# GenkiK/monodepth2

Hardware: AMD Instinct MI355X
Metric: training images/sec at 640x192 mono, 1/2/4/8 GPUs; loss delta vs ref (higher is better)
Workload: dtype f32; 1 GPU; mono_640x192 ResNet-18 batch=12/GPU full train step (configs[1]); global_batch=12, height=192, width=640, parallelism=dp1, step=hipgraph replay

## Files before the change

### include/md2hot.h

```cpp
#ifndef MD2HOT_H
#define MD2HOT_H

#include <stddef.h>
#include <stdint.h>

#ifdef __cplusplus
extern "C" {
#endif

#define MD2_ABI_VERSION 24
#define MD2_MAX_SCALES 4
#define MD2_MAX_SRC 3

#define MD2_OK 0
#define MD2_ERR_ARG (-1)
#define MD2_ERR_HIP (-2)

#define MD2_NO_SSIM          (1u << 0)
#define MD2_AVG_REPROJECTION (1u << 1)
#define MD2_NO_AUTOMASK      (1u << 2)
#define MD2_V1_MULTISCALE    (1u << 3)
#define MD2_T_PER_SCALE      (1u << 4)
#define MD2_PREDICTIVE_MASK  (1u << 5)

// ... 165 lines not shown
    uint8_t reserved;
    uint8_t order[4];
    float brightness, contrast, saturation;
} md2_aug_item;

typedef struct md2_aug_plan md2_aug_plan;

md2_aug_plan* md2_aug_plan_create(const md2_aug_desc* desc);
void md2_aug_plan_destroy(md2_aug_plan* plan);

int md2_aug_run(md2_aug_plan* plan, const uint8_t* frames, const md2_aug_item* items,
                float* const* color, float* const* color_aug, void* stream);
int md2_aug_run2(md2_aug_plan* plan, const uint8_t* frames, const md2_aug_item* items,
                 float* const* color, float* const* color_aug, uint32_t* src8, void* stream);

md2_aug_plan* md2_aug_plan_create_mixed(const md2_aug_desc* desc, const int32_t* sizes, int num_sizes);
int md2_aug_run_mixed(md2_aug_plan* plan, const uint8_t* frames_base, uint64_t total_bytes,
                      const int32_t* item_class, const uint64_t* frame_offset, const md2_aug_item* items,
                      float* const* color, float* const* color_aug, uint32_t* src8, void* stream);

#define MD2_BN_RELU     (1u << 0)
#define MD2_BN_RESIDUAL (1u << 1)
#define MD2_BN_BF16     (1u << 2)

typedef struct md2_bn_desc {
    int64_t pixels;
    int32_t channels;
    uint32_t flags;
    float eps, momentum;
    int32_t groups;
    int32_t reserved;
} md2_bn_desc;

size_t md2_bn_workspace_bytes(const md2_bn_desc* desc);
int md2_bn_fwd(const md2_bn_desc* desc, const void* x, const float* gamma, const float* beta,
               const void* residual, float* running_mean, float* running_var, void* y,
               float* save_mean, float* save_invstd, void* workspace, void* stream);
int md2_bn_bwd(const md2_bn_desc* desc, const void* x, const void* y, const void* grad_y,
               const float* gamma, const float* save_mean, const float* save_invstd,
               void* grad_x, void* grad_residual, float* grad_gamma, float* grad_beta,
               void* workspace, void* stream);
int md2_bn_bwd_multi(const md2_bn_desc* desc, const void* x, const void* y, const void* grad_y,
                     const void* grad_y2, const void* grad_y3, const float* gamma, const float* save_mean,
                     const float* save_invstd, void* grad_x, void* grad_residual, float* grad_gamma,
                     float* grad_beta, void* workspace, void* stream);
int md2_bn_fwd_mask(const md2_bn_desc* desc, const void* x, const float* gamma, const float* beta,
// ... 116 lines not shown

typedef struct md2_viz_desc {
    int32_t batch;
    int32_t in_height, in_width;
    int32_t out_height, out_width;
    int32_t percentile;
    uint32_t flags;
    int32_t reserved;
} md2_viz_desc;

size_t md2_disp_colorize_workspace_bytes(const md2_viz_desc* desc);
int md2_disp_colorize(const md2_viz_desc* desc, const float* disp, uint8_t* rgb, float* resized, float* stats,
                      void* workspace, void* stream);

int md2_bn_pool_fwd_supported(const md2_bn_desc* desc, int height, int width);
int md2_bn_pool_fwd(const md2_bn_desc* desc, int height, int width, const float* x, const float* gamma,
                    const float* beta, float* running_mean, float* running_var, float* y, uint8_t* relu_mask,
                    float* pooled, uint32_t* idx, float* save_mean, float* save_invstd, void* workspace,
                    void* stream);
int md2_bn_bwd_reduce_mask(const md2_bn_desc* desc, const void* x, const uint8_t* relu_mask, const void* grad_y,
                           const float* gamma, const float* save_mean, const float* save_invstd, float* grad_gamma,
                           float* grad_beta, void* workspace, void* stream);
size_t md2_bn_coef_offset(const md2_bn_desc* desc);
int md2_stem_wgrad_bn_supported(const md2_stem_desc* desc);
int md2_stem_wgrad_bn(const md2_stem_desc* desc, const float* x, const float* grad, const float* z,
                      const uint8_t* relu_mask, const float* save_mean, const float* coef, int bn_groups,
                      float* grad_weight, void* workspace, void* stream);

#define MD2_DEPTH16_POST_PROCESS (1u << 0)

typedef struct md2_depth16_desc {
    int32_t batch;
    int32_t in_height, in_width;
    int32_t out_height, out_width;
    uint32_t flags;
    double min_depth, max_depth;
    double scale_factor;
    double clip_max;
    double quant;
    int64_t reserved;
} md2_depth16_desc;

int md2_depth_export16_check(const md2_depth16_desc* desc);
int md2_depth_export16(const md2_depth16_desc* desc, const float* disp, const float* disp_flipped, uint16_t* out,
                       void* stream);

// ... 5 lines not shown
```

### monodepth2_amd/_lib.py

```python
from __future__ import annotations

import ctypes
import os
import threading

import torch

from .build import LIB_PATH as _BUILT_LIB
from .build import source_hash

LIB_PATH = os.environ.get("MD2_LIB", _BUILT_LIB)

MAX_SCALES = 4
MAX_SRC = 3
ABI_VERSION = 24

NO_SSIM = 1 << 0
AVG_REPROJECTION = 1 << 1
NO_AUTOMASK = 1 << 2
V1_MULTISCALE = 1 << 3
T_PER_SCALE = 1 << 4
PREDICTIVE_MASK = 1 << 5

_vp = ctypes.c_void_p
# ... 23 lines not shown
_lib = None

EXPORTS = ["md2_abi_version", "md2_last_error", "md2_workspace_bytes", "md2_select_bytes",
           "md2_photometric_fwd", "md2_photometric_bwd", "md2_generate_images", "md2_tiebreak_noise",
           "md2_timing_begin", "md2_timing_end", "md2_timing_calls", "md2_decoder_pad_fwd", "md2_decoder_pad_bwd",
           "md2_decoder_pad_workspace_bytes", "md2_adam_step", "md2_adam_step_dev", "md2_adam_hyper", "md2_adam_apply_dev", "md2_encoder_input",
           "md2_pose_fwd", "md2_pose_bwd", "md2_aug_plan_create", "md2_aug_plan_destroy", "md2_aug_run",
           "md2_bn_workspace_bytes", "md2_bn_fwd", "md2_bn_bwd", "md2_maxpool3s2_fwd", "md2_maxpool3s2_bwd",
           "md2_disp_head_workspace_bytes", "md2_disp_head_fwd", "md2_disp_head_bwd",
           "md2_stem_wgrad_workspace_bytes", "md2_stem_wgrad", "md2_stem_fwd", "md2_conv_col2im", "md2_bias_act_fwd", "md2_bias_act_bwd",
           "md2_bias_act_workspace_bytes", "md2_maxpool3s2_bwd_add", "md2_bn_bwd_multi",
           "md2_conv_fwd", "md2_conv_workspace_bytes", "md2_conv_split_weights",
           "md2_conv_dgrad", "md2_conv_wgrad", "md2_conv_direct", "md2_conv_wgrad_direct",
           "md2_conv_wgrad_direct_workspace_bytes", "md2_conv_split_weights_multi", "md2_bn_fwd_mask",
           "md2_bn_bwd_mask", "md2_build_id", "md2_maxpool3s2_bwd_multi", "md2_decoder_pad_bwd2", "md2_aug_run2",
           "md2_conv_bf16_weights", "md2_conv_bf16_weights_multi",
           "md2_depth_eval", "md2_depth_eval_workspace_bytes",
           "md2_velo_project", "md2_velo_project_workspace_bytes",
           "md2_pose_ate", "md2_pose_ate_workspace_bytes",
           "md2_disp_colorize", "md2_disp_colorize_workspace_bytes",
           "md2_bn_pool_fwd_supported", "md2_bn_pool_fwd", "md2_bn_bwd_reduce_mask", "md2_bn_coef_offset",
           "md2_stem_wgrad_bn_supported", "md2_stem_wgrad_bn",
           "md2_aug_plan_create_mixed", "md2_aug_run_mixed",
           "md2_depth_export16", "md2_depth_export16_check"]

DTYPE_F32 = 0
DTYPE_BF16 = 1
PAD_ELU = 1 << 0
PAD_UPSAMPLE = 1 << 1
PAD_NHWC = 1 << 2
PAD_BF16 = 1 << 3


class PadDesc(ctypes.Structure):
    _fields_ = [("batch", ctypes.c_int32), ("channels", ctypes.c_int32), ("height", ctypes.c_int32),
                ("width", ctypes.c_int32), ("skip_channels", ctypes.c_int32), ("flags", ctypes.c_uint32)]


class AugDesc(ctypes.Structure):
    _fields_ = [("items", ctypes.c_int32), ("frames", ctypes.c_int32), ("in_height", ctypes.c_int32),
                ("in_width", ctypes.c_int32), ("height", ctypes.c_int32), ("width", ctypes.c_int32),
                ("num_scales", ctypes.c_int32), ("reserved", ctypes.c_int32)]


class AugItem(ctypes.Structure):
    _fields_ = [("flip", ctypes.c_uint8), ("color_aug", ctypes.c_uint8), ("hue_shift", ctypes.c_uint8),
                ("reserved", ctypes.c_uint8), ("order", ctypes.c_uint8 * 4), ("brightness", ctypes.c_float),
                ("contrast", ctypes.c_float), ("saturation", ctypes.c_float)]


BN_RELU = 1 << 0
BN_RESIDUAL = 1 << 1
BN_BF16 = 1 << 2


class BnDesc(ctypes.Structure):
    _fields_ = [("pixels", ctypes.c_int64), ("channels", ctypes.c_int32), ("flags", ctypes.c_uint32),
                ("eps", ctypes.c_float), ("momentum", ctypes.c_float), ("groups", ctypes.c_int32),
                ("reserved", ctypes.c_int32)]


POOL_BF16 = 1 << 0


CONV_NO_SPLIT = 1 << 1
CONV_TILE_N32 = 1 << 2
CONV_TILE_N64 = 1 << 3
CONV_TILE_N128 = 1 << 4
CONV_X6 = 1 << 5
CONV_BM256 = 1 << 6
CONV_PRESPLIT = 1 << 7
CONV_PATCH = 1 << 8
CONV_S2_ONE = 1 << 9
CONV_WS = 1 << 10
CONV_BF16 = 1 << 11

# ... 70 lines not shown

class PoseAteDesc(ctypes.Structure):
    _fields_ = [("sequences", ctypes.c_int32), ("track_length", ctypes.c_int32), ("flags", ctypes.c_uint32),
                ("reserved0", ctypes.c_int32), ("total_frames", ctypes.c_int64), ("reserved", ctypes.c_int64)]


class VizDesc(ctypes.Structure):
    _fields_ = [("batch", ctypes.c_int32), ("in_height", ctypes.c_int32), ("in_width", ctypes.c_int32),
                ("out_height", ctypes.c_int32), ("out_width", ctypes.c_int32), ("percentile", ctypes.c_int32),
                ("flags", ctypes.c_uint32), ("reserved", ctypes.c_int32)]


DEPTH16_POST_PROCESS = 1 << 0


class Depth16Desc(ctypes.Structure):
    _fields_ = [("batch", ctypes.c_int32), ("in_height", ctypes.c_int32), ("in_width", ctypes.c_int32),
                ("out_height", ctypes.c_int32), ("out_width", ctypes.c_int32), ("flags", ctypes.c_uint32),
                ("min_depth", ctypes.c_double), ("max_depth", ctypes.c_double), ("scale_factor", ctypes.c_double),
                ("clip_max", ctypes.c_double), ("quant", ctypes.c_double), ("reserved", ctypes.c_int64)]


def _declare(L):
    L.md2_depth_export16.restype = ctypes.c_int
    L.md2_depth_export16.argtypes = [ctypes.POINTER(Depth16Desc)] + [_vp] * 4
    L.md2_depth_export16_check.restype = ctypes.c_int
    L.md2_depth_export16_check.argtypes = [ctypes.POINTER(Depth16Desc)]
    L.md2_bn_pool_fwd_supported.restype = ctypes.c_int
    L.md2_bn_pool_fwd_supported.argtypes = [ctypes.POINTER(BnDesc), ctypes.c_int, ctypes.c_int]
    L.md2_bn_pool_fwd.restype = ctypes.c_int
    L.md2_bn_pool_fwd.argtypes = [ctypes.POINTER(BnDesc), ctypes.c_int, ctypes.c_int] + [_vp] * 13
    L.md2_bn_bwd_reduce_mask.restype = ctypes.c_int
    L.md2_bn_bwd_reduce_mask.argtypes = [ctypes.POINTER(BnDesc)] + [_vp] * 10
    L.md2_bn_coef_offset.restype = ctypes.c_size_t
    L.md2_bn_coef_offset.argtypes = [ctypes.POINTER(BnDesc)]
    L.md2_stem_wgrad_bn_supported.restype = ctypes.c_int
    L.md2_stem_wgrad_bn_supported.argtypes = [ctypes.POINTER(StemDesc)]
    L.md2_stem_wgrad_bn.restype = ctypes.c_int
    L.md2_stem_wgrad_bn.argtypes = [ctypes.POINTER(StemDesc)] + [_vp] * 6 + [ctypes.c_int] + [_vp] * 3
    L.md2_disp_colorize_workspace_bytes.restype = ctypes.c_size_t
    L.md2_disp_colorize_workspace_bytes.argtypes = [ctypes.POINTER(VizDesc)]
    L.md2_disp_colorize.restype = ctypes.c_int
    L.md2_disp_colorize.argtypes = [ctypes.POINTER(VizDesc)] + [_vp] * 6
    L.md2_pose_ate_workspace_bytes.restype = ctypes.c_size_t
    L.md2_pose_ate_workspace_bytes.argtypes = [ctypes.POINTER(PoseAteDesc)]
    L.md2_pose_ate.restype = ctypes.c_int
# ... 199 lines not shown
```

### monodepth2_amd/csrc/bnorm.hip

```cpp

#include <hip/hip_runtime.h>

#include <stdint.h>
#include <stdlib.h>

#include "md2_bf16.h"
#include "md2_bn_expr.h"
#include "md2hot.h"

int md2_report_error(int code, const char* msg);

namespace {

constexpr int kThreads = 256;
constexpr int kMaxBlocks = 1024;

struct Map {
    int Q;
    int QPT;
    int PPB;
};

__host__ __device__ inline Map make_map(int C) {
    Map m;
    m.Q = C / 4;
    m.QPT = m.Q > kThreads ? m.Q / kThreads : 1;
    m.PPB = m.Q >= kThreads ? 1 : kThreads / m.Q;
// ... 8 lines not shown
__host__ __device__ __forceinline__ Work work(void* ws, int G, int C, int NG) {
    Work w;
    w.part = (float*)ws;
    w.coef = w.part + 2 * (size_t)NG * G * C;
    return w;
}

__device__ __forceinline__ float4 ld4(const float* p) { return *(const float4*)p; }
__device__ __forceinline__ void st4(float* p, float4 v) { *(float4*)p = v; }

template <typename T>
__device__ __forceinline__ float4 ldT(const void* p, size_t off) { return md2::ld4T<T>(p, off); }
template <typename T>
__device__ __forceinline__ void stT(void* p, size_t off, float4 v) { md2::st4T<T>(p, off, v); }

__device__ void block_partials(float4 a, float4 b, int q, int pl, const Map& m, int C, int rows, int row, Work w,
                               float4 (*lds)[kThreads]) {
    lds[0][threadIdx.x] = a;
    lds[1][threadIdx.x] = b;
    __syncthreads();
    for (int half = m.PPB / 2; half > 0; half /= 2) {
        if (pl < half) {
            const int o = threadIdx.x + half * m.Q;
            const float4 u = lds[0][o], v = lds[1][o];
            a.x += u.x; a.y += u.y; a.z += u.z; a.w += u.w;
            b.x += v.x; b.y += v.y; b.z += v.z; b.w += v.w;
            lds[0][threadIdx.x] = a;
            lds[1][threadIdx.x] = b;
        }
        __syncthreads();
    }
    if (pl == 0) {
        float* pa = w.part + (size_t)(4 * q) * rows + row;
        float* pb = w.part + ((size_t)C + 4 * q) * rows + row;
        pa[0] = a.x; pa[rows] = a.y; pa[2 * (size_t)rows] = a.z; pa[3 * (size_t)rows] = a.w;
        pb[0] = b.x; pb[rows] = b.y; pb[2 * (size_t)rows] = b.z; pb[3 * (size_t)rows] = b.w;
    }
    __syncthreads();
}

template <typename T>
__global__ void __launch_bounds__(kThreads) bn_stats_kernel(const void* __restrict__ x, long long P, int C, int G,
                                                            void* ws) {
    const Map m = make_map(C);
    const int NG = gridDim.y, grp = blockIdx.y;
    const Work w = work(ws, G, C, NG);
    x = (const char*)x + (size_t)grp * P * C * sizeof(T);
    __shared__ float4 lds[2][kThreads];
    for (int qq = 0; qq < m.QPT; ++qq) {
        const int q = (threadIdx.x % m.Q) + qq * kThreads, pl = threadIdx.x / m.Q;
        float4 s = {0.f, 0.f, 0.f, 0.f}, ss = {0.f, 0.f, 0.f, 0.f};
        auto acc = [&](const float4 v) {
            s.x += v.x; s.y += v.y; s.z += v.z; s.w += v.w;
            ss.x += v.x * v.x; ss.y += v.y * v.y; ss.z += v.z * v.z; ss.w += v.w * v.w;
        };
        const long long stride = (long long)G * m.PPB;
        long long p = (long long)blockIdx.x * m.PPB + pl;
        for (; p + 3 * stride < P; p += 4 * stride) {
            const float4 v0 = ldT<T>(x, p * C + 4 * q), v1 = ldT<T>(x, (p + stride) * C + 4 * q),
                         v2 = ldT<T>(x, (p + 2 * stride) * C + 4 * q), v3 = ldT<T>(x, (p + 3 * stride) * C + 4 * q);
            acc(v0); acc(v1); acc(v2); acc(v3);
        }
        for (; p < P; p += stride) acc(ldT<T>(x, p * C + 4 * q));
        block_partials(s, ss, q, pl, m, C, NG * G, grp * G + blockIdx.x, w, lds);
    }
}

__device__ bool channel_sums(Work w, int rows, int r0, int G, int C, int c, double& a, double& b) {
    __shared__ double red[2][kThreads / 64];
    static_assert(kMaxBlocks <= 4 * kThreads, "four partial rows per thread at most");
    const float* ca = w.part + (size_t)c * rows + r0;
    const float* cb = w.part + ((size_t)C + c) * rows + r0;
    float pa[4], pb[4];
#pragma unroll
    for (int u = 0; u < 4; ++u) {
        const int g = threadIdx.x + u * kThreads;
        pa[u] = g < G ? ca[g] : 0.f;
        pb[u] = g < G ? cb[g] : 0.f;
    }
    a = 0.0;
    b = 0.0;
#pragma unroll
    for (int u = 0; u < 4; ++u) {
        a += pa[u];
        b += pb[u];
    }
#pragma unroll
    for (int o = 32; o > 0; o >>= 1) {
        a += __shfl_xor(a, o, 64);
        b += __shfl_xor(b, o, 64);
    }
    if ((threadIdx.x & 63) == 0) {
        red[0][threadIdx.x >> 6] = a;
        red[1][threadIdx.x >> 6] = b;
    }
    __syncthreads();
    a = red[0][0];
    b = red[1][0];
#pragma unroll
    for (int i = 1; i < kThreads / 64; ++i) {
        a += red[0][i];
        b += red[1][i];
    }
    __syncthreads();
    return threadIdx.x == 0;
}

__global__ void __launch_bounds__(kThreads) bn_stats_final_kernel(long long P, int C, int G, int NG, float eps,
                                                                  float momentum, float* __restrict__ rmean,
                                                                  float* __restrict__ rvar,
                                                                  float* __restrict__ smean,
                                                                  float* __restrict__ sinvstd, void* ws) {
    const int c = blockIdx.x;
    const Work w = work(ws, G, C, NG);
    for (int grp = 0; grp < NG; ++grp) {
        double a, b;
        if (!channel_sums(w, NG * G, grp * G, G, C, c, a, b)) continue;
        const double mean = a / (double)P;
        double var = b / (double)P - mean * mean;
        var = var > 0.0 ? var : 0.0;
        smean[grp * C + c] = (float)mean;
        sinvstd[grp * C + c] = (float)(1.0 / sqrt(var + (double)eps));
        if (rmean) {
            rmean[c] = (float)((1.0 - momentum) * rmean[c] + momentum * mean);
            rvar[c] = (float)((1.0 - momentum) * rvar[c] + momentum * var * (double)P / (double)(P - 1));
        }
    }
}

template <typename T>
__device__ __forceinline__ bool stored_pos(float o) {
    if constexpr (sizeof(T) == 4) return o > 0.f;
    else return md2::bf2f(md2::f2bf(o)) > 0.f;
}

template <typename T, bool RELU, bool RES, bool MOUT = false>
__global__ void __launch_bounds__(kThreads) bn_apply_kernel(const void* __restrict__ x, const void* __restrict__ r,
                                                            const float* __restrict__ gamma,
                                                            const float* __restrict__ beta,
                                                            const float* __restrict__ smean,
                                                            const float* __restrict__ sinvstd, void* __restrict__ y,
                                                            int n4g, int Q, uint8_t* __restrict__ mask = nullptr) {
    const size_t base = (size_t)blockIdx.y * n4g;
    const float* mug = smean + (size_t)blockIdx.y * 4 * Q;
    const float* isg = sinvstd + (size_t)blockIdx.y * 4 * Q;
    for (int j = blockIdx.x * kThreads + threadIdx.x; j < n4g; j += gridDim.x * kThreads) {
        const size_t i = base + j;
        const int c = 4 * (j & (Q - 1));
// ... 34 lines not shown
    if (g3) {
        const float4 u = ldT<T>(g3, off);
        v.x += u.x; v.y += u.y; v.z += u.z; v.w += u.w;
    }
    return v;
}

template <typename T, bool RELU, bool MIN = false>
__global__ void __launch_bounds__(kThreads) bn_bwd_reduce_kernel(const void* __restrict__ x,
                                                                 const void* __restrict__ y,
                                                                 const void* __restrict__ g,
                                                                 const void* __restrict__ g2,
                                                                 const void* __restrict__ g3, long long P, int C,
                                                                 int G, const float* __restrict__ smean, void* ws) {
    const Map m = make_map(C);
    const int NG = gridDim.y, grp = blockIdx.y;
    const Work w = work(ws, G, C, NG);
    const size_t base = (size_t)grp * P * C;
    __shared__ float4 lds[2][kThreads];
    for (int qq = 0; qq < m.QPT; ++qq) {
        const int q = (threadIdx.x % m.Q) + qq * kThreads, pl = threadIdx.x / m.Q;
        const float4 mu = ld4(smean + grp * C + 4 * q);
        float4 s = {0.f, 0.f, 0.f, 0.f}, sx = {0.f, 0.f, 0.f, 0.f};
        auto acc = [&](float4 gv, const float4 v) {
            s.x += gv.x; s.y += gv.y; s.z += gv.z; s.w += gv.w;
            sx.x += gv.x * (v.x - mu.x); sx.y += gv.y * (v.y - mu.y);
            sx.z += gv.z * (v.z - mu.z); sx.w += gv.w * (v.w - mu.w);
        };
        const long long stride = (long long)G * m.PPB;
        long long p = (long long)blockIdx.x * m.PPB + pl;
        for (; p + stride < P; p += 2 * stride) {
            const size_t o0 = base + p * C + 4 * q, o1 = base + (p + stride) * C + 4 * q;
            float4 g0 = ld_grad<T>(g, g2, g3, o0), g1 = ld_grad<T>(g, g2, g3, o1);
            if (RELU) {
                g0 = relu_gate<T, MIN>(y, o0, g0);
                g1 = relu_gate<T, MIN>(y, o1, g1);
            }
            const float4 v0 = ldT<T>(x, o0), v1 = ldT<T>(x, o1);
            acc(g0, v0);
            acc(g1, v1);
        }
        for (; p < P; p += stride) {
            const size_t o = base + p * C + 4 * q;
            float4 gv = ld_grad<T>(g, g2, g3, o);
            if (RELU) gv = relu_gate<T, MIN>(y, o, gv);
            acc(gv, ldT<T>(x, o));
        }
        block_partials(s, sx, q, pl, m, C, NG * G, grp * G + blockIdx.x, w, lds);
    }
}

__global__ void __launch_bounds__(kThreads) bn_bwd_final_kernel(long long P, int C, int G, int NG,
                                                                const float* __restrict__ gamma,
                                                                const float* __restrict__ sinvstd,
                                                                float* __restrict__ dgamma, float* __restrict__ dbeta,
                                                                void* ws) {
    const int c = blockIdx.x;
    const Work w = work(ws, G, C, NG);
    double sdg = 0.0, sdb = 0.0;
    for (int grp = 0; grp < NG; ++grp) {
        double a, b;
        if (!channel_sums(w, NG * G, grp * G, G, C, c, a, b)) continue;
        const double is = sinvstd[grp * C + c];
        const double dg = b * is;
        sdg += dg;
        sdb += a;
        const size_t gc = (size_t)grp * C + c;
        w.coef[gc] = (float)((double)gamma[c] * is);
        w.coef[(size_t)NG * C + gc] = (float)(a / (double)P);
        w.coef[2 * (size_t)NG * C + gc] = (float)(dg * is / (double)P);
    }
    if (threadIdx.x == 0) {
        dgamma[c] = (float)sdg;
        dbeta[c] = (float)sdb;
    }
}

template <typename T, bool RELU, bool RES, bool MIN = false>
__global__ void __launch_bounds__(kThreads) bn_bwd_apply_kernel(const void* __restrict__ x,
                                                                const void* __restrict__ y,
                                                                const void* __restrict__ g,
                                                                const void* __restrict__ g2,
                                                                const void* __restrict__ g3,
                                                                const float* __restrict__ smean, const float* coef,
                                                                void* __restrict__ dx, void* __restrict__ dr,
                                                                int n4g, int Q, int C, int NG) {
    const size_t base = (size_t)blockIdx.y * n4g;
    const size_t gc = (size_t)blockIdx.y * C;
    for (int j = blockIdx.x * kThreads + threadIdx.x; j < n4g; j += gridDim.x * kThreads) {
        const size_t i = base + j;
        const size_t c = gc + 4 * (j & (Q - 1));
        float4 gv = ld_grad<T>(g, g2, g3, 4 * i);
        if (RELU) gv = relu_gate<T, MIN>(y, 4 * i, gv);
        const float4 v = ldT<T>(x, 4 * i), mu = ld4(smean + c), k1 = ld4(coef + c),
                     k2 = ld4(coef + (size_t)NG * C + c), k3 = ld4(coef + 2 * (size_t)NG * C + c);
        const float4 o = md2::bn_bwd_dx4(gv, v, mu, k1, k2, k3);
        stT<T>(dx, 4 * i, o);
        if (RES) stT<T>(dr, 4 * i, gv);
    }
}

__device__ __forceinline__ void ld8bf(const void* p, size_t off, float (&v)[8]) {
    const uint4 r = *(const uint4*)((const uint16_t*)p + off);
    const uint32_t w[4] = {r.x, r.y, r.z, r.w};
#pragma unroll
    for (int i = 0; i < 4; ++i) {
        v[2 * i] = md2::bf2f(w[i] & 0xffffu);
        v[2 * i + 1] = md2::bf2f(w[i] >> 16);
    }
}
__device__ __forceinline__ void st8bf(void* p, size_t off, const float (&v)[8]) {
    *(uint4*)((uint16_t*)p + off) =
        make_uint4(md2::f2bf(v[0]) | (md2::f2bf(v[1]) << 16), md2::f2bf(v[2]) | (md2::f2bf(v[3]) << 16),
                   md2::f2bf(v[4]) | (md2::f2bf(v[5]) << 16), md2::f2bf(v[6]) | (md2::f2bf(v[7]) << 16));
}
__device__ __forceinline__ void ld8f(const float* p, float (&v)[8]) {
    const float4 a = ld4(p), b = ld4(p + 4);
    v[0] = a.x; v[1] = a.y; v[2] = a.z; v[3] = a.w; v[4] = b.x; v[5] = b.y; v[6] = b.z; v[7] = b.w;
}

template <bool RELU, bool RES, bool MOUT = false>
__global__ void __launch_bounds__(kThreads) bn_apply8_kernel(const void* __restrict__ x, const void* __restrict__ r,
                                                             const float* __restrict__ gamma,
                                                             const float* __restrict__ beta,
// ... 196 lines not shown

int blocks_for_stats(long long P, int C) {
    const Map m = make_map(C);
    const long long rows = (P + m.PPB - 1) / m.PPB;
    const long long g = (rows + 7) / 8;
    return (int)(g < 1 ? 1 : (g > kMaxBlocks ? kMaxBlocks : g));
}

int grid_elem(long long n4, int NG) {
    const long long cap = (4096 + NG - 1) / NG;
    const long long g = (n4 + kThreads - 1) / kThreads;
    return (int)(g < cap ? g : cap);
}

int groups_of(const md2_bn_desc* d) { return d->groups > 1 ? d->groups : 1; }

bool valid(const md2_bn_desc* d) {
    if (!d || d->channels < 4 || d->channels % 4) return false;
    if (d->groups < 0 || d->pixels % groups_of(d) || d->pixels / groups_of(d) < 2) return false;
    const int Q = d->channels / 4;
    if ((Q & (Q - 1)) != 0) return false;
    if ((long long)d->pixels / groups_of(d) * Q >= (1ll << 31)) return false;
    return Q >= kThreads ? (Q % kThreads == 0) : (kThreads % Q == 0);
}

struct StemPoolGeom {
    int B, H, W, Ho, Wo;
    int ipg;
};

template <bool YOUT>
__global__ void __launch_bounds__(kThreads) bn_relu_pool_kernel(StemPoolGeom p, int q_shift,
                                                                const float* __restrict__ z,
                                                                const float* __restrict__ gamma,
                                                                const float* __restrict__ beta,
                                                                const float* __restrict__ smean,
                                                                const float* __restrict__ sinvstd,
                                                                float* __restrict__ y, uint8_t* __restrict__ mask,
                                                                float* __restrict__ pooled,
                                                                uint32_t* __restrict__ idx) {
    const int Q = 1 << q_shift, C = 4 * Q;
    const int j = blockIdx.x * kThreads + threadIdx.x;
    if (j >= p.Wo * Q) return;
    const int row = blockIdx.y, b = row / p.Ho, oy = row - b * p.Ho;
    const int c = 4 * (j & (Q - 1)), ox = j >> q_shift;
    const int gc = (b / p.ipg) * C + c;
// ... 29 lines not shown
}

template <typename T>
void launch_stats(const md2_bn_desc* d, const void* x, float* running_mean, float* running_var, float* save_mean,
                  float* save_invstd, void* workspace, hipStream_t st) {
    const int NG = groups_of(d);
    const long long P = d->pixels / NG;
    const int C = d->channels, G = blocks_for_stats(P, C);
    if (sizeof(T) == 2 && C % 8 == 0 && C <= 8 * kThreads && reduce8_on())
        hipLaunchKernelGGL(bn_stats8_kernel<>, dim3(G, NG), dim3(kThreads), 0, st, x, P, C, G, workspace);
    else
        hipLaunchKernelGGL(bn_stats_kernel<T>, dim3(G, NG), dim3(kThreads), 0, st, x, P, C, G, workspace);
    hipLaunchKernelGGL(bn_stats_final_kernel, dim3(C), dim3(kThreads), 0, st, P, C, G, NG, d->eps, d->momentum,
                       running_mean, running_var, save_mean, save_invstd, workspace);
}

template <typename T>
void launch_fwd(const md2_bn_desc* d, const void* x, const float* gamma, const float* beta, const void* residual,
                float* running_mean, float* running_var, void* y, float* save_mean, float* save_invstd,
                void* workspace, hipStream_t st, uint8_t* mask = nullptr) {
    const int NG = groups_of(d);
    const long long P = d->pixels / NG;
    const int C = d->channels;
    launch_stats<T>(d, x, running_mean, running_var, save_mean, save_invstd, workspace, st);
    const int n4g = (int)(P * C / 4);
    const bool relu = d->flags & MD2_BN_RELU, res = d->flags & MD2_BN_RESIDUAL;
    if (sizeof(T) == 2 && C % 8 == 0 && apply8_on()) {
        auto k8 = relu ? (mask ? (res ? bn_apply8_kernel<true, true, true> : bn_apply8_kernel<true, false, true>)
                               : (res ? bn_apply8_kernel<true, true> : bn_apply8_kernel<true, false>))
                       : (res ? bn_apply8_kernel<false, true> : bn_apply8_kernel<false, false>);
        hipLaunchKernelGGL(k8, dim3(grid_elem(n4g / 2, NG), NG), dim3(kThreads), 0, st, x, residual, gamma, beta,
                           save_mean, save_invstd, y, n4g / 2, C / 8, mask);
        return;
    }
    auto k = relu ? (mask ? (res ? bn_apply_kernel<T, true, true, true> : bn_apply_kernel<T, true, false, true>)
                          : (res ? bn_apply_kernel<T, true, true> : bn_apply_kernel<T, true, false>))
                  : (res ? bn_apply_kernel<T, false, true> : bn_apply_kernel<T, false, false>);
    hipLaunchKernelGGL(k, dim3(grid_elem(n4g, NG), NG), dim3(kThreads), 0, st, x, residual, gamma, beta, save_mean,
                       save_invstd, y, n4g, C / 4, mask);
}

template <typename T>
void launch_bwd_reduce(const md2_bn_desc* d, const void* x, const void* y, const void* grad_y, const void* grad_y2,
                       const void* grad_y3, const float* gamma, const float* save_mean, const float* save_invstd,
                       float* grad_gamma, float* grad_beta, void* workspace, hipStream_t st, bool mask_in) {
    const int NG = groups_of(d);
    const long long P = d->pixels / NG;
    const int C = d->channels, G = blocks_for_stats(P, C);
    const bool relu = d->flags & MD2_BN_RELU;
    auto red = relu ? (mask_in ? bn_bwd_reduce_kernel<T, true, true> : bn_bwd_reduce_kernel<T, true>)
                    : bn_bwd_reduce_kernel<T, false>;
    if (sizeof(T) == 2 && C % 8 == 0 && C <= 8 * kThreads && reduce8_on())
        red = relu ? (mask_in ? bn_bwd_reduce8_kernel<true, true> : bn_bwd_reduce8_kernel<true>)
                   : bn_bwd_reduce8_kernel<false>;
    hipLaunchKernelGGL(red, dim3(G, NG), dim3(kThreads), 0, st, x, y, grad_y, grad_y2, grad_y3, P, C, G, save_mean,
                       workspace);
    hipLaunchKernelGGL(bn_bwd_final_kernel, dim3(C), dim3(kThreads), 0, st, P, C, G, NG, gamma, save_invstd,
                       grad_gamma, grad_beta, workspace);
}

template <typename T>
void launch_bwd(const md2_bn_desc* d, const void* x, const void* y, const void* grad_y, const void* grad_y2,
                const void* grad_y3, const float* gamma,
                const float* save_mean, const float* save_invstd, void* grad_x, void* grad_residual,
                float* grad_gamma, float* grad_beta, void* workspace, hipStream_t st, bool mask_in = false) {
    const int NG = groups_of(d);
    const long long P = d->pixels / NG;
    const int C = d->channels, G = blocks_for_stats(P, C);
    const bool relu = d->flags & MD2_BN_RELU, res = d->flags & MD2_BN_RESIDUAL;
    launch_bwd_reduce<T>(d, x, y, grad_y, grad_y2, grad_y3, gamma, save_mean, save_invstd, grad_gamma, grad_beta,
                         workspace, st, mask_in);
    const int n4g = (int)(P * C / 4);
    const float* coef = work(workspace, G, C, NG).coef;
    if (sizeof(T) == 2 && C % 8 == 0 && apply8_on()) {
        auto k8 = relu ? (mask_in ? (res ? bn_bwd_apply8_kernel<true, true, true> : bn_bwd_apply8_kernel<true, false, true>)
                                  : (res ? bn_bwd_apply8_kernel<true, true> : bn_bwd_apply8_kernel<true, false>))
                       : (res ? bn_bwd_apply8_kernel<false, true> : bn_bwd_apply8_kernel<false, false>);
        hipLaunchKernelGGL(k8, dim3(grid_elem(n4g / 2, NG), NG), dim3(kThreads), 0, st, x, y, grad_y, grad_y2,
                           grad_y3, save_mean, coef, grad_x, grad_residual, n4g / 2, C / 8, C, NG);
        return;
    }
    auto k = relu ? (mask_in ? (res ? bn_bwd_apply_kernel<T, true, true, true> : bn_bwd_apply_kernel<T, true, false, true>)
                             : (res ? bn_bwd_apply_kernel<T, true, true> : bn_bwd_apply_kernel<T, true, false>))
                  : (res ? bn_bwd_apply_kernel<T, false, true> : bn_bwd_apply_kernel<T, false, false>);
    hipLaunchKernelGGL(k, dim3(grid_elem(n4g, NG), NG), dim3(kThreads), 0, st, x, y, grad_y, grad_y2, grad_y3,
                       save_mean, coef, grad_x, grad_residual, n4g, C / 4, C, NG);
}

}

extern "C" {

// ... 109 lines not shown
                       gamma, beta, save_mean, save_invstd, y, relu_mask, pooled, idx);
    const hipError_t e = hipGetLastError();
    return e == hipSuccess ? MD2_OK : md2_report_error(MD2_ERR_HIP, hipGetErrorString(e));
}

int md2_bn_bwd_reduce_mask(const md2_bn_desc* d, const void* x, const uint8_t* relu_mask, const void* grad_y,
                           const float* gamma, const float* save_mean, const float* save_invstd, float* grad_gamma,
                           float* grad_beta, void* workspace, void* stream) {
    if (!valid(d)) return md2_report_error(MD2_ERR_ARG, "bn: unsupported shape");
    if (!(d->flags & MD2_BN_RELU)) return md2_report_error(MD2_ERR_ARG, "bn_bwd_reduce_mask: needs MD2_BN_RELU");
    if (!x || !relu_mask || !grad_y || !gamma || !save_mean || !save_invstd || !grad_gamma || !grad_beta ||
        !workspace)
        return md2_report_error(MD2_ERR_ARG, "bn_bwd_reduce_mask: NULL operand");
    if (d->flags & MD2_BN_BF16)
        launch_bwd_reduce<uint16_t>(d, x, relu_mask, grad_y, nullptr, nullptr, gamma, save_mean, save_invstd,
                                    grad_gamma, grad_beta, workspace, (hipStream_t)stream, true);
    else
        launch_bwd_reduce<float>(d, x, relu_mask, grad_y, nullptr, nullptr, gamma, save_mean, save_invstd,
                                 grad_gamma, grad_beta, workspace, (hipStream_t)stream, true);
    const hipError_t e = hipGetLastError();
    return e == hipSuccess ? MD2_OK : md2_report_error(MD2_ERR_HIP, hipGetErrorString(e));
}

size_t md2_bn_coef_offset(const md2_bn_desc* d) {
    if (!valid(d)) return 0;
    const int NG = groups_of(d);
    const int G = blocks_for_stats(d->pixels / NG, d->channels);
    return 2 * (size_t)NG * G * d->channels * sizeof(float);
}

int md2_bn_bwd(const md2_bn_desc* d, const void* x, const void* y, const void* grad_y, const float* gamma,
               const float* save_mean, const float* save_invstd, void* grad_x, void* grad_residual,
               float* grad_gamma, float* grad_beta, void* workspace, void* stream) {
    return md2_bn_bwd_multi(d, x, y, grad_y, nullptr, nullptr, gamma, save_mean, save_invstd, grad_x, grad_residual,
                            grad_gamma, grad_beta, workspace, stream);
}

}
```

### monodepth2_amd/csrc/md2_bn_expr.h

```cpp
#pragma once

#include <hip/hip_runtime.h>

#include <stdint.h>

namespace md2 {

__device__ __forceinline__ float4 bn_affine4(const float4 v, const float4 mu, const float4 is, const float4 ga,
                                             const float4 be) {
    float4 o;
    o.x = (v.x - mu.x) * is.x * ga.x + be.x;
    o.y = (v.y - mu.y) * is.y * ga.y + be.y;
    o.z = (v.z - mu.z) * is.z * ga.z + be.z;
    o.w = (v.w - mu.w) * is.w * ga.w + be.w;
    return o;
}

__device__ __forceinline__ float4 relu4(float4 o) {
    o.x = fmaxf(o.x, 0.f); o.y = fmaxf(o.y, 0.f); o.z = fmaxf(o.z, 0.f); o.w = fmaxf(o.w, 0.f);
    return o;
}

__device__ __forceinline__ float4 relu_gate_bits4(const uint32_t m, float4 g) {
    g.x = (m & 1) ? g.x : 0.f; g.y = (m & 2) ? g.y : 0.f; g.z = (m & 4) ? g.z : 0.f; g.w = (m & 8) ? g.w : 0.f;
    return g;
}
__device__ __forceinline__ float4 relu_gate_mask4(const void* mask, size_t off, float4 g) {
    return relu_gate_bits4(((const uint8_t*)mask)[off >> 2], g);
}

__device__ __forceinline__ float4 bn_bwd_dx4(const float4 gv, const float4 v, const float4 mu, const float4 k1,
                                             const float4 k2, const float4 k3) {
    float4 o;
    o.x = k1.x * (gv.x - k2.x - (v.x - mu.x) * k3.x);
    o.y = k1.y * (gv.y - k2.y - (v.y - mu.y) * k3.y);
    o.z = k1.z * (gv.z - k2.z - (v.z - mu.z) * k3.z);
    o.w = k1.w * (gv.w - k2.w - (v.w - mu.w) * k3.w);
    return o;
}

__device__ __forceinline__ void pool_take(float v, int k, float& m, int& a) {
    if (v > m || isnan(v)) {
        m = v;
        a = k;
    }
}

}
```

Before: 1148 images/s.

## Add single-kernel batchnorm path for small deep layers with LDS stashing

Measured after the change: 1148 images/s. No clear change (-0.0%).

```diff
diff --git a/include/md2hot.h b/include/md2hot.h
--- a/include/md2hot.h
+++ b/include/md2hot.h
@@ -211,6 +211,7 @@
 #define MD2_BN_RELU     (1u << 0)
 #define MD2_BN_RESIDUAL (1u << 1)
 #define MD2_BN_BF16     (1u << 2)
+#define MD2_BN_THREE_PASS (1u << 3)
 
 typedef struct md2_bn_desc {
     int64_t pixels;
@@ -373,6 +374,8 @@
                            const float* gamma, const float* save_mean, const float* save_invstd, float* grad_gamma,
                            float* grad_beta, void* workspace, void* stream);
 size_t md2_bn_coef_offset(const md2_bn_desc* desc);
+void md2_bn_small_limits(int min_channels, long long max_bytes);
+long long md2_bn_small_calls(void);
 int md2_stem_wgrad_bn_supported(const md2_stem_desc* desc);
 int md2_stem_wgrad_bn(const md2_stem_desc* desc, const float* x, const float* grad, const float* z,
                       const uint8_t* relu_mask, const float* save_mean, const float* coef, int bn_groups,
diff --git a/monodepth2_amd/_lib.py b/monodepth2_amd/_lib.py
--- a/monodepth2_amd/_lib.py
+++ b/monodepth2_amd/_lib.py
@@ -69,7 +69,8 @@
            "md2_bn_pool_fwd_supported", "md2_bn_pool_fwd", "md2_bn_bwd_reduce_mask", "md2_bn_coef_offset",
            "md2_stem_wgrad_bn_supported", "md2_stem_wgrad_bn",
            "md2_aug_plan_create_mixed", "md2_aug_run_mixed",
-           "md2_depth_export16", "md2_depth_export16_check"]
+           "md2_depth_export16", "md2_depth_export16_check",
+           "md2_bn_small_limits", "md2_bn_small_calls"]
 
 DTYPE_F32 = 0
 DTYPE_BF16 = 1
@@ -99,6 +100,7 @@
 BN_RELU = 1 << 0
 BN_RESIDUAL = 1 << 1
 BN_BF16 = 1 << 2
+BN_THREE_PASS = 1 << 3
 
 
 class BnDesc(ctypes.Structure):
@@ -215,6 +217,10 @@
 
 
 def _declare(L):
+    L.md2_bn_small_limits.restype = None
+    L.md2_bn_small_limits.argtypes = [ctypes.c_int, ctypes.c_longlong]
+    L.md2_bn_small_calls.restype = ctypes.c_longlong
+    L.md2_bn_small_calls.argtypes = []
     L.md2_depth_export16.restype = ctypes.c_int
     L.md2_depth_export16.argtypes = [ctypes.POINTER(Depth16Desc)] + [_vp] * 4
     L.md2_depth_export16_check.restype = ctypes.c_int
diff --git a/monodepth2_amd/csrc/bnorm.hip b/monodepth2_amd/csrc/bnorm.hip
--- a/monodepth2_amd/csrc/bnorm.hip
+++ b/monodepth2_amd/csrc/bnorm.hip
@@ -3,6 +3,8 @@
 
 #include <stdint.h>
 #include <stdlib.h>
+
+#include <atomic>
 
 #include "md2_bf16.h"
 #include "md2_bn_expr.h"
@@ -57,9 +59,7 @@
     for (int half = m.PPB / 2; half > 0; half /= 2) {
         if (pl < half) {
             const int o = threadIdx.x + half * m.Q;
-            const float4 u = lds[0][o], v = lds[1][o];
-            a.x += u.x; a.y += u.y; a.z += u.z; a.w += u.w;
-            b.x += v.x; b.y += v.y; b.z += v.z; b.w += v.w;
+            md2::bn_lane_add(a, b, lds[0][o], lds[1][o]);
             lds[0][threadIdx.x] = a;
             lds[1][threadIdx.x] = b;
         }
@@ -85,10 +85,7 @@
     for (int qq = 0; qq < m.QPT; ++qq) {
         const int q = (threadIdx.x % m.Q) + qq * kThreads, pl = threadIdx.x / m.Q;
         float4 s = {0.f, 0.f, 0.f, 0.f}, ss = {0.f, 0.f, 0.f, 0.f};
-        auto acc = [&](const float4 v) {
-            s.x += v.x; s.y += v.y; s.z += v.z; s.w += v.w;
-            ss.x += v.x * v.x; ss.y += v.y * v.y; ss.z += v.z * v.z; ss.w += v.w * v.w;
-        };
+        auto acc = [&](const float4 v) { md2::bn_acc_stats(s, ss, v); };
         const long long stride = (long long)G * m.PPB;
         long long p = (long long)blockIdx.x * m.PPB + pl;
         for (; p + 3 * stride < P; p += 4 * stride) {
@@ -106,37 +103,13 @@
     static_assert(kMaxBlocks <= 4 * kThreads, "four partial rows per thread at most");
     const float* ca = w.part + (size_t)c * rows + r0;
     const float* cb = w.part + ((size_t)C + c) * rows + r0;
-    float pa[4], pb[4];
-#pragma unroll
-    for (int u = 0; u < 4; ++u) {
-        const int g = threadIdx.x + u * kThreads;
-        pa[u] = g < G ? ca[g] : 0.f;
-        pb[u] = g < G ? cb[g] : 0.f;
-    }
-    a = 0.0;
-    b = 0.0;
-#pragma unroll
-    for (int u = 0; u < 4; ++u) {
-        a += pa[u];
-        b += pb[u];
-    }
-#pragma unroll
-    for (int o = 32; o > 0; o >>= 1) {
-        a += __shfl_xor(a, o, 64);
-        b += __shfl_xor(b, o, 64);
-    }
+    md2::bn_rows_wave_sums<kThreads>(ca, cb, G, a, b);
     if ((threadIdx.x & 63) == 0) {
         red[0][threadIdx.x >> 6] = a;
         red[1][threadIdx.x >> 6] = b;
     }
     __syncthreads();
-    a = red[0][0];
-    b = red[1][0];
-#pragma unroll
-    for (int i = 1; i < kThreads / 64; ++i) {
-        a += red[0][i];
-        b += red[1][i];
-    }
+    md2::bn_wave_fold<kThreads / 64>(red[0], red[1], a, b);
     __syncthreads();
     return threadIdx.x == 0;
 }
@@ -151,14 +124,13 @@
     for (int grp = 0; grp < NG; ++grp) {
         double a, b;
         if (!channel_sums(w, NG * G, grp * G, G, C, c, a, b)) continue;
-        const double mean = a / (double)P;
-        double var = b / (double)P - mean * mean;
-        var = var > 0.0 ? var : 0.0;
+        double mean, var;
+        md2::bn_mean_var(a, b, P, mean, var);
         smean[grp * C + c] = (float)mean;
-        sinvstd[grp * C + c] = (float)(1.0 / sqrt(var + (double)eps));
+        sinvstd[grp * C + c] = md2::bn_invstd(var, eps);
         if (rmean) {
-            rmean[c] = (float)((1.0 - momentum) * rmean[c] + momentum * mean);
-            rvar[c] = (float)((1.0 - momentum) * rvar[c] + momentum * var * (double)P / (double)(P - 1));
+            rmean[c] = md2::bn_running_mean(rmean[c], momentum, mean);
+            rvar[c] = md2::bn_running_var(rvar[c], momentum, var, P);
         }
     }
 }
@@ -239,11 +211,7 @@
         const int q = (threadIdx.x % m.Q) + qq * kThreads, pl = threadIdx.x / m.Q;
         const float4 mu = ld4(smean + grp * C + 4 * q);
         float4 s = {0.f, 0.f, 0.f, 0.f}, sx = {0.f, 0.f, 0.f, 0.f};
-        auto acc = [&](float4 gv, const float4 v) {
-            s.x += gv.x; s.y += gv.y; s.z += gv.z; s.w += gv.w;
-            sx.x += gv.x * (v.x - mu.x); sx.y += gv.y * (v.y - mu.y);
-            sx.z += gv.z * (v.z - mu.z); sx.w += gv.w * (v.w - mu.w);
-        };
+        auto acc = [&](float4 gv, const float4 v) { md2::bn_acc_bwd(s, sx, gv, v, mu); };
         const long long stride = (long long)G * m.PPB;
         long long p = (long long)blockIdx.x * m.PPB + pl;
         for (; p + stride < P; p += 2 * stride) {
@@ -279,13 +247,13 @@
         double a, b;
         if (!channel_sums(w, NG * G, grp * G, G, C, c, a, b)) continue;
         const double is = sinvstd[grp * C + c];
-        const double dg = b * is;
+        const double dg = md2::bn_bwd_dgamma(b, is);
         sdg += dg;
         sdb += a;
         const size_t gc = (size_t)grp * C + c;
-        w.coef[gc] = (float)((double)gamma[c] * is);
-        w.coef[(size_t)NG * C + gc] = (float)(a / (double)P);
-        w.coef[2 * (size_t)NG * C + gc] = (float)(dg * is / (double)P);
+        w.coef[gc] = md2::bn_bwd_k1(gamma[c], is);
+        w.coef[(size_t)NG * C + gc] = md2::bn_bwd_k2(a, P);
+        w.coef[2 * (size_t)NG * C + gc] = md2::bn_bwd_k3(dg, is, P);
     }
     if (threadIdx.x == 0) {
         dgamma[c] = (float)sdg;
@@ -317,6 +285,235 @@
     }
 }
 
+constexpr int kSmallRows = 512;
+
+struct SmallLds {
+    float rows[8][kSmallRows];
+    double red[8][kThreads / 64];
+    float fin[12];
+};
+
+__device__ __forceinline__ int small_quad(int Q) {
+    const int b = blockIdx.x;
+    return Q % 8 == 0 ? (b & 7) * (Q >> 3) + (b >> 3) : b;
+}
+
+__device__ __forceinline__ void small_fold_lanes(float4 a, float4 b, int vl, int stride, int PPB, SmallLds& L) {
+    for (int half = PPB / 2; half > 0; half /= 2) {
+        float4 u, v;
+        u.x = __shfl_down(a.x, half, 64); u.y = __shfl_down(a.y, half, 64);
+        u.z = __shfl_down(a.z, half, 64); u.w = __shfl_down(a.w, half, 64);
+        v.x = __shfl_down(b.x, half, 64); v.y = __shfl_down(b.y, half, 64);
+        v.z = __shfl_down(b.z, half, 64); v.w = __shfl_down(b.w, half, 64);
+        md2::bn_lane_add(a, b, u, v);
+    }
+    if (vl < stride && (vl & (PPB - 1)) == 0) {
+        const int bx = vl / PPB;
+        L.rows[0][bx] = a.x; L.rows[1][bx] = a.y; L.rows[2][bx] = a.z; L.rows[3][bx] = a.w;
+        L.rows[4][bx] = b.x; L.rows[5][bx] = b.y; L.rows[6][bx] = b.z; L.rows[7][bx] = b.w;
+    }
+}
+
+__device__ __forceinline__ void small_wave_sums(int G, SmallLds& L) {
+#pragma unroll
+    for (int j = 0; j < 4; ++j) {
+        double a, b;
+        md2::bn_rows_wave_sums<kThreads>(L.rows[j], L.rows[4 + j], G, a, b);
+        if ((threadIdx.x & 63) == 0) {
+            L.red[j][threadIdx.x >> 6] = a;
+            L.red[4 + j][threadIdx.x >> 6] = b;
+        }
+    }
+}
+
+template <bool RELU, bool RES, bool STASH>
+__global__ void __launch_bounds__(kThreads) bn_small_fwd_kernel(const float* __restrict__ x, const float* __restrict__ r,
+                                                                const float* __restrict__ gamma,
+                                                                const float* __restrict__ beta,
+                                                                float* __restrict__ rmean, float* __restrict__ rvar,
+                                                                float* __restrict__ smean,
+                                                                float* __restrict__ sinvstd, float* __restrict__ y,
+                                                                uint8_t* __restrict__ mask, int P, int C, int G,
+                                                                int NG, float eps, float momentum) {
+    extern __shared__ float4 col[];
+    __shared__ SmallLds L;
+    const Map m = make_map(C);
+    const int q = small_quad(m.Q), t = threadIdx.x;
+    const int stride = G * m.PPB;
+    const float4 ga = ld4(gamma + 4 * q), be = ld4(beta + 4 * q);
+    for (int grp = 0; grp < NG; ++grp) {
+        const size_t base = (size_t)grp * P * C + 4 * q;
+        for (int v0 = 0; v0 < stride; v0 += kThreads) {
+            const int vl = v0 + t;
+            float4 s = {0.f, 0.f, 0.f, 0.f}, ss = {0.f, 0.f, 0.f, 0.f};
+            if (vl < stride) {
+                for (int p = vl; p < P; p += 4 * stride) {
+                    float4 v[4];
+#pragma unroll
+                    for (int u = 0; u < 4; ++u) {
+                        const int pu = p + u * stride;
+                        v[u] = ld4(x + base + (size_t)(pu < P ? pu : p) * C);
+                    }
+#pragma unroll
+                    for (int u = 0; u < 4; ++u) {
+                        const int pu = p + u * stride;
+                        if (pu < P) {
+                            md2::bn_acc_stats(s, ss, v[u]);
+                            if (STASH) col[pu] = v[u];
+                        }
+                    }
+                }
+            }
+            small_fold_lanes(s, ss, vl, stride, m.PPB, L);
+        }
+        __syncthreads();
+        small_wave_sums(G, L);
+        __syncthreads();
+        if (t < 4) {
+            const int c = 4 * q + t;
+            double a, b, mean, var;
+            md2::bn_wave_fold<kThreads / 64>(L.red[t], L.red[4 + t], a, b);
+            md2::bn_mean_var(a, b, P, mean, var);
+            const float mf = (float)mean, isf = md2::bn_invstd(var, eps);
+            smean[grp * C + c] = mf;
+            sinvstd[grp * C + c] = isf;
+            if (rmean) {
+                rmean[c] = md2::bn_running_mean(rmean[c], momentum, mean);
+                rvar[c] = md2::bn_running_var(rvar[c], momentum, var, P);
+            }
+            L.fin[t] = mf;
+            L.fin[4 + t] = isf;
+        }
+        __syncthreads();
+        const float4 mu = make_float4(L.fin[0], L.fin[1], L.fin[2], L.fin[3]),
+                     is = make_float4(L.fin[4], L.fin[5], L.fin[6], L.fin[7]);
+        for (int p = t; p < P; p += 4 * kThreads) {
+            float4 v[4], rv[4];
+#pragma unroll
+            for (int u = 0; u < 4; ++u) {
+                const int pu = p + u * kThreads, pc = pu < P ? pu : p;
+                v[u] = STASH ? col[pc] : ld4(x + base + (size_t)pc * C);
+                if (RES) rv[u] = ld4(r + base + (size_t)pc * C);
+            }
+#pragma unroll
+            for (int u = 0; u < 4; ++u) {
+                const int pu = p + u * kThreads;
+                if (pu >= P) continue;
+                const size_t e = base + (size_t)pu * C;
+                float4 o = md2::bn_affine4(v[u], mu, is, ga, be);
+                if (RES) {
+                    o.x += rv[u].x; o.y += rv[u].y; o.z += rv[u].z; o.w += rv[u].w;
+                }
+                if (RELU) o = md2::relu4(o);
+                st4(y + e, o);
+                if (RELU)
+                    mask[e >> 2] = (uint8_t)((stored_pos<float>(o.x) ? 1 : 0) | (stored_pos<float>(o.y) ? 2 : 0) |
+                                             (stored_pos<float>(o.z) ? 4 : 0) | (stored_pos<float>(o.w) ? 8 : 0));
+            }
+        }
+        __syncthreads();
+    }
+}
+
+template <bool RELU, bool RES, bool STASH>
+__global__ void __launch_bounds__(kThreads) bn_small_bwd_kernel(const float* __restrict__ x,
+                                                                const uint8_t* __restrict__ mask,
+                                                                const float* __restrict__ g,
+                                                                const float* __restrict__ g2,
+                                                                const float* __restrict__ g3,
+                                                                const float* __restrict__ gamma,
+                                                                const float* __restrict__ smean,
+                                                                const float* __restrict__ sinvstd,
+                                                                float* __restrict__ dx, float* __restrict__ dr,
+                                                                float* __restrict__ dgamma, float* __restrict__ dbeta,
+                                                                int P, int C, int G, int NG, bool stash_x) {
+    extern __shared__ float4 col[];
+    __shared__ SmallLds L;
+    const Map m = make_map(C);
+    const int q = small_quad(m.Q), t = threadIdx.x;
+    const int stride = G * m.PPB;
+    double sdg = 0.0, sdb = 0.0;
+    auto grad = [&](size_t e) {
+        float4 gv = ld_grad<float>(g, g2, g3, e);
+        if (RELU) gv = relu_gate<float, true>(mask, e, gv);
+        return gv;
+    };
+    for (int grp = 0; grp < NG; ++grp) {
+        const size_t base = (size_t)grp * P * C + 4 * q;
+        const float4 mu = ld4(smean + grp * C + 4 * q);
+        for (int v0 = 0; v0 < stride; v0 += kThreads) {
+            const int vl = v0 + t;
+            float4 s = {0.f, 0.f, 0.f, 0.f}, sx = {0.f, 0.f, 0.f, 0.f};
+            if (vl < stride) {
+                for (int p = vl; p < P; p += 4 * stride) {
+                    float4 gv[4], v[4];
+#pragma unroll
+                    for (int u = 0; u < 4; ++u) {
+                        const int pu = p + u * stride;
+                        const size_t e = base + (size_t)(pu < P ? pu : p) * C;
+                        gv[u] = grad(e);
+                        v[u] = ld4(x + e);
+                    }
+#pragma unroll
+                    for (int u = 0; u < 4; ++u) {
+                        const int pu = p + u * stride;
+                        if (pu < P) {
+                            md2::bn_acc_bwd(s, sx, gv[u], v[u], mu);
+                            if (STASH) {
+                                col[pu] = gv[u];
+                                if (stash_x) col[P + pu] = v[u];
+                            }
+                        }
+                    }
+                }
+            }
+            small_fold_lanes(s, sx, vl, stride, m.PPB, L);
+        }
+        __syncthreads();
+        small_wave_sums(G, L);
+        __syncthreads();
+        if (t < 4) {
+            const int c = 4 * q + t;
+            double a, b;
+            md2::bn_wave_fold<kThreads / 64>(L.red[t], L.red[4 + t], a, b);
+            const double is = sinvstd[grp * C + c];
+            const double dg = md2::bn_bwd_dgamma(b, is);
+            sdg += dg;
+            sdb += a;
+            L.fin[t] = md2::bn_bwd_k1(gamma[c], is);
+            L.fin[4 + t] = md2::bn_bwd_k2(a, P);
+            L.fin[8 + t] = md2::bn_bwd_k3(dg, is, P);
+        }
+        __syncthreads();
+        const float4 k1 = make_float4(L.fin[0], L.fin[1], L.fin[2], L.fin[3]),
+                     k2 = make_float4(L.fin[4], L.fin[5], L.fin[6], L.fin[7]),
+                     k3 = make_float4(L.fin[8], L.fin[9], L.fin[10], L.fin[11]);
+        for (int p = t; p < P; p += 4 * kThreads) {
+            float4 gv[4], v[4];
+#pragma unroll
+            for (int u = 0; u < 4; ++u) {
+                const int pu = p + u * kThreads, pc = pu < P ? pu : p;
+                const size_t e = base + (size_t)pc * C;
+                gv[u] = STASH ? col[pc] : grad(e);
+                v[u] = STASH && stash_x ? col[P + pc] : ld4(x + e);
+            }
+#pragma unroll
+            for (int u = 0; u < 4; ++u) {
+                const int pu = p + u * kThreads;
+                if (pu >= P) continue;
+                const size_t e = base + (size_t)pu * C;
+                st4(dx + e, md2::bn_bwd_dx4(gv[u], v[u], mu, k1, k2, k3));
+                if (RES) st4(dr + e, gv[u]);
+            }
+        }
+        __syncthreads();
+    }
+    if (t < 4) {
+        dgamma[4 * q + t] = (float)sdg;
+        dbeta[4 * q + t] = (float)sdb;
+    }
+}
+
 __device__ __forceinline__ void ld8bf(const void* p, size_t off, float (&v)[8]) {
     const uint4 r = *(const uint4*)((const uint16_t*)p + off);
     const uint32_t w[4] = {r.x, r.y, r.z, r.w};
@@ -559,6 +756,96 @@
     if ((Q & (Q - 1)) != 0) return false;
     if ((long long)d->pixels / groups_of(d) * Q >= (1ll << 31)) return false;
     return Q >= kThreads ? (Q % kThreads == 0) : (kThreads % Q == 0);
+}
+
+constexpr int kSmallCmin = 512;
+constexpr long long kSmallMaxBytes = 3ll << 20;
+std::atomic<int> g_small_cmin{kSmallCmin};
+std::atomic<long long> g_small_max_bytes{kSmallMaxBytes};
+std::atomic<long long> g_small_calls{0};
+
+int small_mode() {
+    static const int mode = [] {
+        const char* e = getenv("MD2_BN_SMALL");
+        return e && e[0] == '0' ? 0 : (e && e[0] == '2' ? 2 : 1);
+    }();
+    return mode;
+}
+
+int lds_per_block() {
+    static const int bytes = [] {
+        int dev = 0, v = 0;
+        if (hipGetDevice(&dev) != hipSuccess ||
+            hipDeviceGetAttribute(&v, hipDeviceAttributeMaxSharedMemoryPerBlock, dev) != hipSuccess || v < 65536)
+            v = 65536;
+        return v;
+    }();
+    return bytes;
+}
+
+bool small_ok(const md2_bn_desc* d, bool relu_by_mask) {
+    if (small_mode() == 0 || (d->flags & (MD2_BN_BF16 | MD2_BN_THREE_PASS))) return false;
+    const bool relu = d->flags & MD2_BN_RELU, res = d->flags & MD2_BN_RESIDUAL;
+    if (relu ? !relu_by_mask : res) return false;
+    const int C = d->channels, Q = C / 4;
+    if (Q >= kThreads || kThreads / Q > 64) return false;
+    if (blocks_for_stats(d->pixels / groups_of(d), C) > kSmallRows) return false;
+    return C >= g_small_cmin.load() && d->pixels * C * (long long)sizeof(float) <= g_small_max_bytes.load();
+}
+
+size_t small_stash_bytes(const void* kernel, std::atomic<bool>& told, long long P, int columns = 1) {
+    const size_t need = (size_t)columns * P * sizeof(float4), room = (size_t)lds_per_block() - sizeof(SmallLds) - 256;
+    if (small_mode() == 2 || need > room) return 0;
+    if (need > 48 * 1024 && !told.load()) {
+        if (hipFuncSetAttribute(kernel, hipFuncAttributeMaxDynamicSharedMemorySize, (int)room) != hipSuccess) {
+            (void)hipGetLastError();
+            return 0;
+        }
+        told.store(true);
+    }
+    return need;
+}
+
+bool launch_small_fwd(const md2_bn_desc* d, const float* x, const float* gamma, const float* beta, const float* r,
+                      float* rmean, float* rvar, float* y, float* smean, float* sinvstd, hipStream_t st,
+                      uint8_t* mask) {
+    if (!small_ok(d, mask != nullptr)) return false;
+    const int NG = groups_of(d), C = d->channels;
+    const int P = (int)(d->pixels / NG), G = blocks_for_stats(P, C);
+    const int form = (d->flags & MD2_BN_RELU) ? ((d->flags & MD2_BN_RESIDUAL) ? 2 : 1) : 0;
+    static std::atomic<bool> told[3];
+    using K = decltype(&bn_small_fwd_kernel<false, false, false>);
+    static const K plain[3] = {bn_small_fwd_kernel<false, false, false>, bn_small_fwd_kernel<true, false, false>,
+                               bn_small_fwd_kernel<true, true, false>};
+    static const K stash[3] = {bn_small_fwd_kernel<false, false, true>, bn_small_fwd_kernel<true, false, true>,
+                               bn_small_fwd_kernel<true, true, true>};
+    const size_t lds = small_stash_bytes((const void*)stash[form], told[form], P);
+    hipLaunchKernelGGL(lds ? stash[form] : plain[form], dim3(C / 4), dim3(kThreads), lds, st, x, r, gamma, beta, rmean,
+                       rvar, smean, sinvstd, y, mask, P, C, G, NG, d->eps, d->momentum);
+    g_small_calls.fetch_add(1);
+    return true;
+}
+
+bool launch_small_bwd(const md2_bn_desc* d, const float* x, const uint8_t* mask, const float* g, const float* g2,
+                      const float* g3, const float* gamma, const float* smean, const float* sinvstd, float* dx,
+                      float* dr, float* dgamma, float* dbeta, hipStream_t st, bool mask_in) {
+    if (!small_ok(d, mask_in)) return false;
+    const int NG = groups_of(d), C = d->channels;
+    const int P = (int)(d->pixels / NG), G = blocks_for_stats(P, C);
+    const int form = (d->flags & MD2_BN_RELU) ? ((d->flags & MD2_BN_RESIDUAL) ? 2 : 1) : 0;
+    static std::atomic<bool> told[3];
+    using K = decltype(&bn_small_bwd_kernel<false, false, false>);
+    static const K plain[3] = {bn_small_bwd_kernel<false, false, false>, bn_small_bwd_kernel<true, false, false>,
+                               bn_small_bwd_kernel<true, true, false>};
+    static const K stash[3] = {bn_small_bwd_kernel<false, false, true>, bn_small_bwd_kernel<true, false, true>,
+                               bn_small_bwd_kernel<true, true, true>};
+    size_t lds = small_stash_bytes((const void*)stash[form], told[form], P, 2);
+    const bool stash_x = lds != 0;
+    if (!lds) lds = small_stash_bytes((const void*)stash[form], told[form], P);
+    hipLaunchKernelGGL(lds ? stash[form] : plain[form], dim3(C / 4), dim3(kThreads), lds, st, x, mask, g, g2, g3, gamma,
+                       smean, sinvstd, dx, dr, dgamma, dbeta, P, C, G, NG, stash_x);
+    g_small_calls.fetch_add(1);
+    return true;
 }
 
 struct StemPoolGeom {
@@ -634,6 +921,10 @@
     const int NG = groups_of(d);
     const long long P = d->pixels / NG;
     const int C = d->channels;
+    if constexpr (sizeof(T) == 4)
+        if (launch_small_fwd(d, (const float*)x, gamma, beta, (const float*)residual, running_mean, running_var,
+                             (float*)y, save_mean, save_invstd, st, mask))
+            return;
     launch_stats<T>(d, x, running_mean, running_var, save_mean, save_invstd, workspace, st);
     const int n4g = (int)(P * C / 4);
     const bool relu = d->flags & MD2_BN_RELU, res = d->flags & MD2_BN_RESIDUAL;
@@ -680,6 +971,11 @@
     const long long P = d->pixels / NG;
     const int C = d->channels, G = blocks_for_stats(P, C);
     const bool relu = d->flags & MD2_BN_RELU, res = d->flags & MD2_BN_RESIDUAL;
+    if constexpr (sizeof(T) == 4)
+        if (launch_small_bwd(d, (const float*)x, (const uint8_t*)y, (const float*)grad_y, (const float*)grad_y2,
+                             (const float*)grad_y3, gamma, save_mean, save_invstd, (float*)grad_x,
+                             (float*)grad_residual, grad_gamma, grad_beta, st, mask_in))
+            return;
     launch_bwd_reduce<T>(d, x, y, grad_y, grad_y2, grad_y3, gamma, save_mean, save_invstd, grad_gamma, grad_beta,
                          workspace, st, mask_in);
     const int n4g = (int)(P * C / 4);
@@ -835,6 +1131,13 @@
     return e == hipSuccess ? MD2_OK : md2_report_error(MD2_ERR_HIP, hipGetErrorString(e));
 }
 
+void md2_bn_small_limits(int min_channels, long long max_bytes) {
+    g_small_cmin.store(min_channels > 0 ? min_channels : kSmallCmin);
+    g_small_max_bytes.store(max_bytes > 0 ? max_bytes : kSmallMaxBytes);
+}
+
+long long md2_bn_small_calls(void) { return g_small_calls.load(); }
+
 size_t md2_bn_coef_offset(const md2_bn_desc* d) {
     if (!valid(d)) return 0;
     const int NG = groups_of(d);
diff --git a/monodepth2_amd/csrc/md2_bn_expr.h b/monodepth2_amd/csrc/md2_bn_expr.h
--- a/monodepth2_amd/csrc/md2_bn_expr.h
+++ b/monodepth2_amd/csrc/md2_bn_expr.h
@@ -39,6 +39,75 @@
     return o;
 }
 
+
+__device__ __forceinline__ void bn_acc_stats(float4& s, float4& ss, const float4 v) {
+    s.x += v.x; s.y += v.y; s.z += v.z; s.w += v.w;
+    ss.x += v.x * v.x; ss.y += v.y * v.y; ss.z += v.z * v.z; ss.w += v.w * v.w;
+}
+
+__device__ __forceinline__ void bn_acc_bwd(float4& s, float4& sx, const float4 gv, const float4 v, const float4 mu) {
+    s.x += gv.x; s.y += gv.y; s.z += gv.z; s.w += gv.w;
+    sx.x += gv.x * (v.x - mu.x); sx.y += gv.y * (v.y - mu.y);
+    sx.z += gv.z * (v.z - mu.z); sx.w += gv.w * (v.w - mu.w);
+}
+
+__device__ __forceinline__ void bn_lane_add(float4& a, float4& b, const float4 u, const float4 v) {
+    a.x += u.x; a.y += u.y; a.z += u.z; a.w += u.w;
+    b.x += v.x; b.y += v.y; b.z += v.z; b.w += v.w;
+}
+
+template <int THREADS>
+__device__ __forceinline__ void bn_rows_wave_sums(const float* ca, const float* cb, int G, double& a, double& b) {
+    float pa[4], pb[4];
+#pragma unroll
+    for (int u = 0; u < 4; ++u) {
+        const int g = threadIdx.x + u * THREADS;
+        pa[u] = g < G ? ca[g] : 0.f;
+        pb[u] = g < G ? cb[g] : 0.f;
+    }
+    a = 0.0;
+    b = 0.0;
+#pragma unroll
+    for (int u = 0; u < 4; ++u) {
+        a += pa[u];
+        b += pb[u];
+    }
+#pragma unroll
+    for (int o = 32; o > 0; o >>= 1) {
+        a += __shfl_xor(a, o, 64);
+        b += __shfl_xor(b, o, 64);
+    }
+}
+
+template <int WAVES>
+__device__ __forceinline__ void bn_wave_fold(const double* ra, const double* rb, double& a, double& b) {
+    a = ra[0];
+    b = rb[0];
+#pragma unroll
+    for (int i = 1; i < WAVES; ++i) {
+        a += ra[i];
+        b += rb[i];
+    }
+}
+
+__device__ __forceinline__ void bn_mean_var(double a, double b, long long P, double& mean, double& var) {
+    mean = a / (double)P;
+    var = b / (double)P - mean * mean;
+    var = var > 0.0 ? var : 0.0;
+}
+__device__ __forceinline__ float bn_invstd(double var, float eps) { return (float)(1.0 / sqrt(var + (double)eps)); }
+__device__ __forceinline__ float bn_running_mean(float rm, float momentum, double mean) {
+    return (float)((1.0 - momentum) * rm + momentum * mean);
+}
+__device__ __forceinline__ float bn_running_var(float rv, float momentum, double var, long long P) {
+    return (float)((1.0 - momentum) * rv + momentum * var * (double)P / (double)(P - 1));
+}
+
+__device__ __forceinline__ double bn_bwd_dgamma(double b, double is) { return b * is; }
+__device__ __forceinline__ float bn_bwd_k1(float gamma, double is) { return (float)((double)gamma * is); }
+__device__ __forceinline__ float bn_bwd_k2(double a, long long P) { return (float)(a / (double)P); }
+__device__ __forceinline__ float bn_bwd_k3(double dg, double is, long long P) { return (float)(dg * is / (double)P); }
+
 __device__ __forceinline__ void pool_take(float v, int k, float& m, int& a) {
     if (v > m || isnan(v)) {
         m = v;
```
